# MeshFEM/MeshFEM

Measured on AMD Instinct MI355X. Metric: stiffness_assembly_elements_per_s, higher is better.
Workload: dtype f64

## Files before the change

### meshfem_amd/csrc/mfh_api.cpp

```cpp
#include "mfh_ctx.hh"
#include <dlfcn.h>

using namespace mfh;

namespace {
struct RoctxApi {
    int (*push)(const char *) = nullptr;
    int (*pop)() = nullptr;
    RoctxApi() {
        const char *en = getenv("MFH_ROCTX");
        if (!en || en[0] == '0') return;
        for (const char *lib : {"librocprofiler-sdk-roctx.so", "libroctx64.so", "/opt/rocm/lib/librocprofiler-sdk-roctx.so", "/opt/rocm/lib/libroctx64.so"}) {
            if (void *h = dlopen(lib, RTLD_NOW | RTLD_GLOBAL)) {
                push = reinterpret_cast<int (*)(const char *)>(dlsym(h, "roctxRangePushA"));
                pop = reinterpret_cast<int (*)()>(dlsym(h, "roctxRangePop"));
                if (push && pop) return;
                push = nullptr; pop = nullptr;
            }
        }
    }
};
RoctxApi &roctx_api() { static RoctxApi a; return a; }
}
mfh::RoctxRange::RoctxRange(const char *name) {
// ... 67 lines not shown
void upload_mesh(mfh_ctx *c, bool deviceTables) {
    double t0 = now_ms();
    c->autoStretch = -1.0;
    drop_p1_view(c);
    c->opDegree = 0;
    c->nodePairsValid = false;
    if (!c->hostOnly && !deviceTables) {
        require_device(c);
        MFH_HIP(hipSetDevice(c->device));
        c->dElemNodes.upload(c->mesh.elemNodes, c->stream);
        c->dVertPos.upload(c->mesh.nodePos, c->stream);
    }
    c->timing.upload_ms = now_ms() - t0;
    c->haveMesh = true;
    c->external = false;
    c->geoValid = false;
    c->hGeoValid = false;
    c->dofForNode.clear();
    c->nDoF = c->mesh.nNode;
    build_shape_tables(c->mesh.dim, c->mesh.deg, c->tables);
    if (!c->hostOnly) { c->dPairTable.upload(c->tables.pairTable, c->stream); c->dMassTable.upload(c->tables.massRef, c->stream); }
    invalidate_symbolic(c);
    dist_detach(c);
    reset_bcs(c);
    clear_fixed(c);
}

void set_isotropic(mfh_ctx *c, double E, double nu) {
    double lam = (nu * E) / ((1.0 + nu) * (1.0 - 2.0 * nu));
    if (c->haveMesh && c->mesh.dim == 2) lam = (nu * E) / (1.0 - nu * nu);
    c->matMode = 0;
    c->matKind = MAT_ISO;
    c->matParams = {lam, E / (2.0 + 2.0 * nu), E, nu};
    c->geoValid = false;
    c->hGeoValid = false;
    invalidate_matrix(c);
}

void drop_p1_view(mfh_ctx *c) {
    if (c->p1) { mfh_destroy(c->p1); c->p1 = nullptr; }
    c->p1GeoGen = -1;
}

mfh_ctx *p1_view(mfh_ctx *c) {
    if (!c || c->opDegree != 1 || !c->p1) return nullptr;
    mfh_ctx *v = c->p1;
    if (!c->hostOnly) {
        ensure_geometry(c);
        v->dGeo.borrow(c->dGeo.p, c->dGeo.n);
        v->geoStride = c->geoStride;
        v->geoValid = true;
        if (v->dVertPos.borrowed || !v->dVertPos.p) v->dVertPos.borrow(c->dVertPos.p, (size_t)v->mesh.nNode * v->mesh.dim);
        if (c->p1GeoGen != c->geoGen) { invalidate_matrix(v); c->p1GeoGen = c->geoGen; }
    }
    return v;
}

void ensure_pass_events(mfh_ctx *c) {
    if (c->passEv[0]) return;
    for (auto &e : c->passEv) MFH_HIP(hipEventCreate(&e));
    MFH_HIP(hipHostMalloc((void **)&c->negHost, 2 * sizeof(int), hipHostMallocDefault));
}

void ensure_geometry(mfh_ctx *c, bool deferCheck) {
    require(c->haveMesh, MFH_ERR_STATE, "no mesh set");
    if (c->geoValid) return;
    require(!c->hostOnly, MFH_ERR_HIP, "host-only context (device -1): no HIP device, and there is no CPU fallback");
    require_device(c);
    MFH_HIP(hipSetDevice(c->device));
    const HostMesh &m = c->mesh;
    if (c->matParams.empty() && !c->dMatBorrowed) set_isotropic(c, 1.0, 0.3);
    if (c->matMode == 0 && !c->dMatBorrowed) {
        double E = c->matParams[2], nu = c->matParams[3];
        double lam = (nu * E) / ((1.0 + nu) * (1.0 - 2.0 * nu));
        if (m.dim == 2) lam = (nu * E) / (1.0 - nu * nu);
        c->matParams[0] = lam;
    }
    c->geoStride = c->matKind == MAT_ISO ? GEO_ISO_STRIDE : (c->matKind == MAT_ORTHO ? GEO_ORTHO_STRIDE : GEO_GEN_STRIDE);
    if (!c->dMatBorrowed) c->dMatParams.upload(c->matParams, c->stream);
    const double *dMat = c->dMatBorrowed ? c->dMatBorrowed : c->dMatParams.p;
    c->dGeo.alloc((size_t)m.nElem * c->geoStride);
    c->dNeg.alloc(2);
    c->dNeg.zero(c->stream);
    ensure_pass_events(c);
    MFH_HIP(hipEventRecord(c->passEv[0], c->stream));
    k::launch_geometry(m.dim, m.deg, c->matKind, m.nElem, c->dElemNodes.p, m.npe, c->dVertPos.p, dMat, c->matMode,
                       c->dGeo.p, c->geoStride, c->dNeg.p, c->stream);
    MFH_HIP(hipEventRecord(c->passEv[1], c->stream));
    MFH_HIP(hipMemcpyAsync(c->negHost, c->dNeg.p, 2 * sizeof(int), hipMemcpyDeviceToHost, c->stream));
    c->geoPending = true;
    if (!deferCheck) finish_geometry(c);
}

void finish_geometry(mfh_ctx *c) {
    if (!c->geoPending) return;
    c->geoPending = false;
    MFH_HIP(hipStreamSynchronize(c->stream));
    float ms = 0;
    MFH_HIP(hipEventElapsedTime(&ms, c->passEv[0], c->passEv[1]));
    c->timing.geometry_ms = ms;
    const int neg[2] = {c->negHost[0], c->negHost[1]};
    if (neg[0] > 0)
        throw Error(MFH_ERR_INVALID, "Mesh has negatively oriented elements.\nCorrect with: mesh_convert --reorientNegativeElements. (" +
                                         std::to_string(neg[0]) + " elements)");
    if (neg[1] > 0)
        throw Error(MFH_ERR_INVALID, std::string(c->matMode == 1 ? "Isotropic" : "Orthotropic") + " parameters of " + std::to_string(neg[1]) +
                                         " elements give an indefinite elasticity tensor (" +
                                         (c->matMode == 1 ? "need E > 0 and -1 < nu < 1/2, nu < 1 in plane stress" : "compliance matrix not positive definite") + ").");
    c->geoValid = true;
    c->hGeoValid = false;
    ++c->geoGen;
}

const std::vector<double> &host_geo(mfh_ctx *c) {
    ensure_geometry(c);
    if (!c->hGeoValid) {
        c->hGeo.resize(c->dGeo.n);
        c->dGeo.download(c->hGeo.data(), c->dGeo.n, c->stream);
        c->hGeoValid = true;
    }
    return c->hGeo;
}

const int32_t *device_dof_map(mfh_ctx *c) {
    if (c->dofForNode.empty()) return nullptr;
    if (!c->dofUploaded) { c->dDofForNode.upload(c->dofForNode, c->stream); c->dofUploaded = true; }
    return c->dDofForNode.p;
}

void ensure_host_colidx(mfh_ctx *c) {
    if (!c->sym.colIdx.empty() || c->sym.nnzb == 0) return;
    c->sym.colIdx.resize((size_t)c->sym.nnzb);
    c->dColIdx.download(c->sym.colIdx.data(), c->sym.colIdx.size(), c->stream);
}
// ... 1009 lines not shown
    MFH_TRY(c)
    require(c && out, MFH_ERR_INVALID, "null argument");
    const std::vector<double> &g = host_geo(c);
    for (int64_t e = 0; e < c->mesh.nElem; ++e) out[e] = g[(size_t)e * c->geoStride + 12];
    MFH_CATCH(c)
}

mfh_status mfh_material_isotropic(mfh_ctx *c, double E, double nu) {
    MFH_TRY(c)
    require(c, MFH_ERR_INVALID, "null context");
    set_isotropic(c, E, nu);
    MFH_CATCH(c)
}

mfh_status mfh_material_const(mfh_ctx *c, const double *D) {
    MFH_TRY(c)
    require(c && D && c->haveMesh, MFH_ERR_STATE, "set the mesh before the material");
    const int d = c->dim(), fl = flat_len(d);
    c->matParams.clear();
    bool ortho = true;
    for (int r = 0; r < fl && ortho; ++r)
        for (int cc = r + 1; cc < fl; ++cc)
            if (cc >= d && D[r * fl + cc] != 0.0) { ortho = false; break; }
    if (ortho) {
        for (int r = 0; r < d; ++r)
            for (int cc = r; cc < d; ++cc) c->matParams.push_back(D[r * fl + cc]);
        for (int k2 = d; k2 < fl; ++k2) c->matParams.push_back(D[k2 * fl + k2]);
        c->matMode = 5; c->matKind = MAT_ORTHO;
    } else {
        for (int r = 0; r < fl; ++r)
            for (int cc = r; cc < fl; ++cc) c->matParams.push_back(D[r * fl + cc]);
        c->matMode = 2; c->matKind = MAT_GENERAL;
    }
    c->geoValid = false; c->hGeoValid = false;
    invalidate_matrix(c);
    MFH_CATCH(c)
}

mfh_status mfh_material_iso_field(mfh_ctx *c, const double *E, const double *nu) {
    MFH_TRY(c)
    require(c && E && nu && c->haveMesh, MFH_ERR_STATE, "set the mesh before the material");
    const int64_t n = c->mesh.nElem;
    c->matParams.assign((size_t)2 * n, 0.0);
    std::copy(E, E + n, c->matParams.begin());
    std::copy(nu, nu + n, c->matParams.begin() + n);
    c->matMode = 1; c->matKind = MAT_ISO;
    c->geoValid = false; c->hGeoValid = false;
    invalidate_matrix(c);
    MFH_CATCH(c)
}

mfh_status mfh_material_ortho_field(mfh_ctx *c, const double *params) {
    MFH_TRY(c)
    require(c && params && c->haveMesh, MFH_ERR_STATE, "set the mesh before the material");
    const int np = c->dim() == 3 ? 9 : 4;
    c->matParams.assign(params, params + (size_t)np * c->mesh.nElem);
    c->matMode = 3; c->matKind = MAT_ORTHO;
    c->geoValid = false; c->hGeoValid = false;
    invalidate_matrix(c);
    MFH_CATCH(c)
}

mfh_status mfh_material_tensor_field(mfh_ctx *c, const double *D) {
    MFH_TRY(c)
    require(c && D && c->haveMesh, MFH_ERR_STATE, "set the mesh before the material");
    const int fl = flat_len(c->dim());
    c->matParams.assign(D, D + (size_t)fl * fl * c->mesh.nElem);
    c->matMode = 4; c->matKind = MAT_GENERAL;
    c->geoValid = false; c->hGeoValid = false;
    invalidate_matrix(c);
    MFH_CATCH(c)
}

mfh_status mfh_material_get(mfh_ctx *c, int64_t elem, double *D) {
    MFH_TRY(c)
    require(c && D && c->haveMesh && elem >= 0 && elem < c->mesh.nElem, MFH_ERR_INVALID, "bad element");
    const std::vector<double> &g = host_geo(c);
    elem_D(c, &g[(size_t)elem * c->geoStride], D);
    MFH_CATCH(c)
}

mfh_status mfh_dof_map(mfh_ctx *c, const int32_t *dofForNode, int64_t nDoF) {
    MFH_TRY(c)
    require(!(c && c->opDegree == 1 && c->p1), MFH_ERR_STATE, "a forced-degree-1 view is in force (mfh_set_operator_degree): it is defined for the identity DoF map");
    require(c && c->haveMesh, MFH_ERR_STATE, "no mesh set");
    c->nOwnedDoFSet = -1;
    if (!dofForNode) {
        c->dofForNode.clear();
        c->nDoF = c->mesh.nNode;
        std::fill(c->mesh.bdryInternal.begin(), c->mesh.bdryInternal.end(), (uint8_t)0);
    } else {
        require(c->mesh.nOwned == c->mesh.nNode, MFH_ERR_UNSUPPORTED, "a DoF map on a partitioned mesh says which DoFs are this rank's rows: mfh_dof_map_partitioned");
        require(nDoF > 0 && nDoF <= c->mesh.nNode, MFH_ERR_INVALID, "bad nDoF");
        for (int64_t n = 0; n < c->mesh.nNode; ++n)
            require(dofForNode[n] >= 0 && dofForNode[n] < nDoF, MFH_ERR_INVALID, "DoF index out of range");
        c->dofForNode.assign(dofForNode, dofForNode + c->mesh.nNode);
        c->nDoF = nDoF;
    }
    invalidate_symbolic(c);
    clear_fixed(c);
    MFH_CATCH(c)
// ... 58 lines not shown

mfh_status mfh_symbolic_get(const mfh_ctx *c, int32_t *rowPtr, int32_t *colIdx, int32_t *chunkRow, int64_t *contribPtr,
                            uint32_t *contribCode, uint16_t *contribSlot, int32_t *scatterSlot) {
    if (c && c->opDegree == 1 && c->p1) return mfh_symbolic_get(c->p1, rowPtr, colIdx, chunkRow, contribPtr, contribCode, contribSlot, scatterSlot);
    if (!c || !c->symValid) return MFH_ERR_STATE;
    const Symbolic &S = c->sym;
    if (rowPtr) std::copy(S.rowPtr.begin(), S.rowPtr.end(), rowPtr);
    if (colIdx) std::copy(S.colIdx.begin(), S.colIdx.end(), colIdx);
    if (chunkRow) std::copy(S.chunkRow.begin(), S.chunkRow.end(), chunkRow);
    if (contribPtr) std::copy(S.contribPtr.begin(), S.contribPtr.end(), contribPtr);
    if (contribCode || contribSlot || scatterSlot) {
        if (S.contribCode.empty()) return MFH_ERR_STATE;
        if (contribCode) std::copy(S.contribCode.begin(), S.contribCode.end(), contribCode);
        if (contribSlot) std::copy(S.contribSlot.begin(), S.contribSlot.end(), contribSlot);
        if (scatterSlot) {
            if (S.scatterSlot.empty()) return MFH_ERR_STATE;
            std::copy(S.scatterSlot.begin(), S.scatterSlot.end(), scatterSlot);
        }
    }
    return MFH_OK;
}

mfh_status mfh_assemble(mfh_ctx *c, int32_t mode) {
    { mfh_status st; if (follow_view(c, st, [&](mfh_ctx *v) { return mfh_assemble(v, mode); })) return st; }
    MFH_TRY(c)
    require(c && c->haveMesh, MFH_ERR_STATE, "no mesh set");
    require(mode == MFH_ASSEMBLE_GATHER || mode == MFH_ASSEMBLE_ATOMIC, MFH_ERR_INVALID, "bad assembly mode");
    require(!(c->deterministic && mode == MFH_ASSEMBLE_ATOMIC), MFH_ERR_UNSUPPORTED, "option deterministic: the global-atomic assembly variant is not reproducible");
    if (c->alwaysReembed) { c->geoValid = false; c->hGeoValid = false; }
    ensure_symbolic(c, mode == MFH_ASSEMBLE_ATOMIC);
    RoctxRange range("Assemble System");
    ensure_geometry(c, true);
    ensure_pass_events(c);
    MFH_HIP(hipEventRecord(c->passEv[2], c->stream));
    run_assembly(c, mode);
    MFH_HIP(hipEventRecord(c->passEv[3], c->stream));
    if (c->geoPending) finish_geometry(c);
    else MFH_HIP(hipStreamSynchronize(c->stream));
    float ms = 0;
    MFH_HIP(hipEventElapsedTime(&ms, c->passEv[2], c->passEv[3]));
    c->timing.assemble_ms = ms;
    if (mode == MFH_ASSEMBLE_GATHER && c->placementTrials > 0 && c->placementGen != c->valsGen) placement_trials(c);
    c->assembled = true;
    c->dinvValid = false;
    MFH_CATCH(c)
}

mfh_status mfh_matrix_info(const mfh_ctx *c, int64_t *nBlockRows, int64_t *nBlockCols, int64_t *nnzBlocks) {
    if (c && c->opDegree == 1 && c->p1) return mfh_matrix_info(c->p1, nBlockRows, nBlockCols, nnzBlocks);
    if (!c || !c->symValid) return MFH_ERR_STATE;
    if (nBlockRows) *nBlockRows = c->sym.nRows;
    if (nBlockCols) *nBlockCols = c->sym.nCols;
    if (nnzBlocks) *nnzBlocks = c->sym.nnzb + (c->upperOnly ? c->sym.nMirror : 0);
    return MFH_OK;
}

mfh_status mfh_matrix_storage(const mfh_ctx *c, int32_t *upperOnly, int64_t *storedBlocks) {
    if (c && c->opDegree == 1 && c->p1) return mfh_matrix_storage(c->p1, upperOnly, storedBlocks);
    if (!c || !c->symValid) return MFH_ERR_STATE;
    if (upperOnly) *upperOnly = c->upperOnly ? 1 : 0;
    if (storedBlocks) *storedBlocks = c->sym.nnzb;
    return MFH_OK;
}

mfh_status mfh_matrix_set_upper_triplets(mfh_ctx *c, int64_t n, int64_t nnz, const uint64_t *ti, const uint64_t *tj, const double *tv) {
    MFH_TRY(c)
    require(c && n > 0 && nnz >= 0 && (nnz == 0 || (ti && tj && tv)), MFH_ERR_INVALID, "bad matrix arguments");
    require(n < (int64_t)1 << 31, MFH_ERR_UNSUPPORTED, "matrix too large for 32-bit indices");
    require(nnz < ((int64_t)1 << 30), MFH_ERR_UNSUPPORTED, "matrix has too many non-zeros for 32-bit slots (2 nnz must stay below 2^31)");
    require_device(c);
    MFH_HIP(hipSetDevice(c->device));
    struct Ent { int32_t r, c; double v; };
    std::vector<Ent> ent;
// ... 786 lines not shown
```

### meshfem_amd/csrc/mfh_ctx.hh

```
#pragma once
#include "mfh_internal.hh"
#include <cmath>
#include <map>
#include <mutex>

using namespace mfh;

struct mfh_ctx {
    int device = 0;
    bool hostOnly = false;
    bool hierarchyLevel = false;
    bool keepHostSymbolic = false;
    int xcdSwizzle = 0;
    RawVec<double> hLoad, hX, hXBatch, hLoadBatch;
    bool alwaysReembed = false;
    bool deterministic = false;
    DBuf<double> detPartials;
    DBuf<unsigned> detCounter;
    bool periodicIgnoreMismatch = false;
    int periodicIgnoreDims = 0;
    hipStream_t stream = nullptr;
    bool ownStream = true;
    bool arenaCounted = false;
    std::string err;

    HostMesh mesh;
    bool haveMesh = false;
    bool external = false;
    DBuf<int32_t> dElemNodes;
    DBuf<double> dVertPos;

    int matMode = 0;
    int matKind = MAT_ISO;
    int op = MFH_OP_ELASTICITY;
    int opDegree = 0;
    mfh_ctx *p1 = nullptr;
    int64_t geoGen = 0, p1GeoGen = -1;
    DBuf<int32_t> dNodePtr, dNodePair;
    bool nodePairsValid = false;
    std::vector<double> matParams;
    DBuf<double> dMatParams;
    const double *dMatBorrowed = nullptr;
    DBuf<double> dGeo;
    DBuf<int> dNeg;
    int geoStride = GEO_ISO_STRIDE;
    bool geoValid = false;
    hipEvent_t passEv[4] = {nullptr, nullptr, nullptr, nullptr};
    int *negHost = nullptr;
    bool geoPending = false;
    std::vector<double> hGeo;
    bool hGeoValid = false;

    std::vector<int32_t> dofForNode;
    DBuf<int32_t> dDofForNode;
    bool dofUploaded = false;
    int64_t nDoF = 0;

    Symbolic sym;
    bool symValid = false;
    bool symHasScatter = false;
    DBuf<int32_t> dRowPtr, dColIdx, dChunkRow, dSpmvChunkRow, dScatter;
    DBuf<int64_t> dContribPtr;
    int matrixStorage = -1;
    bool upperOnly = false;
    int nCU = 256;
    DBuf<uint32_t> dContribCode;
    DBuf<uint16_t> dContribSlot;
    ShapeTables tables;
    DBuf<double> dPairTable, dMassTable;
    MfLists mf;
    bool mfValid = false;
    int matrixFree = -1;
    bool use_mf() const {
        if (external || !haveMesh || hostOnly || kron()) return false;
        return matrixFree == 1 || (matrixFree < 0 && op == MFH_OP_ELASTICITY);
    }
    DBuf<int32_t> dMfChunkRow;
    DBuf<int64_t> dMfPairPtr;
    DBuf<uint32_t> dMfPairCode, dMfPairPos;
    DBuf<uint16_t> dMfPairRow;
    MfClusterLists mfc;
// ... 242 lines not shown
}

inline bool resolve_upper_storage(const mfh_ctx *c) {
    if (c->matrixStorage >= 0) return c->matrixStorage == 1;
    return c->haveMesh && !c->hostOnly && !c->external && c->op == MFH_OP_ELASTICITY && c->use_mf() && !c->tlProbe && c->tlRapAgg;
}

inline void require_full_storage(const mfh_ctx *c, const char *what) {
    if (c->upperOnly) throw Error(MFH_ERR_UNSUPPORTED, std::string(what) + " needs both triangles of K: set option matrix_storage to 0");
}

inline int32_t dof_of(const mfh_ctx *c, int64_t node) { return c->dofForNode.empty() ? (int32_t)node : c->dofForNode[node]; }
void invalidate_matrix(mfh_ctx *c);
void ensure_dirichlet_tables(mfh_ctx *c);
void dist_detach(mfh_ctx *c);
bool dist_active(const mfh_ctx *c);
int dist_rank(const mfh_ctx *c);
int dist_world(const mfh_ctx *c);
void dist_apply(mfh_ctx *c, double *x, double *y, bool masked);
void dist_halo(mfh_ctx *c, double *v, int W);
void dist_allreduce(mfh_ctx *c, double *dev, int64_t n);
void dist_level_forward(mfh_ctx *c, mfh_ctx::AggLevel &A, double *v, int W);
void dist_level_reverse_add(mfh_ctx *c, mfh_ctx::AggLevel &A, double *v, int W);
void dist_exchange_lists(mfh_ctx *c, const std::vector<std::vector<int32_t>> &toRank, std::vector<std::vector<int32_t>> &fromRank);
void dist_setup_child(mfh_ctx *c, mfh_ctx *child, const std::vector<int32_t> &keep);
void dist_agree(mfh_ctx *c);
void dist_profile_collect(mfh_ctx *c);
void refresh_storage_rule(mfh_ctx *c);
void reset_bcs(mfh_ctx *c);
void clear_fixed(mfh_ctx *c);
void add_fixed(mfh_ctx *c, int64_t n, const int64_t *vars, const double *vals);
void ensure_geometry(mfh_ctx *c, bool deferCheck = false);
void finish_geometry(mfh_ctx *c);
void ensure_node_pairs(mfh_ctx *c);
void ensure_mf_cluster(mfh_ctx *c);
void upload_mesh(mfh_ctx *c, bool deviceTables);
void ensure_fixed_uploaded(mfh_ctx *c);
bool prepare_matrix_free(mfh_ctx *c);
k::SpmvArgs spmv_args(mfh_ctx *c, bool masked);
k::SpmvMfArgs spmv_mf_args(mfh_ctx *c, bool masked);
k::SpmvMfArgs spmv_mf_cluster_args(mfh_ctx *c, bool masked);
k::TLArgs tl_args(mfh_ctx *c);
void apply_operator(mfh_ctx *c, bool masked, const double *x, double *y, double *dotOut);
void apply_operator_smoother(mfh_ctx *c, bool masked, const double *x, double *y);
void batch_apply(mfh_ctx *c, int NR, double *x, double *y, bool masked);
void tl_precond(mfh_ctx *c, const double *r, double *z, double *scal, int it);
bool dense_inverse_device(mfh_ctx *c, const double *Ac, int64_t mm, DBuf<double> &Ainv, int64_t &ldInv);
double device_dot(mfh_ctx *c, int64_t n, const double *a, const double *b);
void ensure_precond(mfh_ctx *c);
bool ensure_twolevel(mfh_ctx *c);
bool ensure_multigrid(mfh_ctx *c);
void ensure_coarse_levels(mfh_ctx *c, int nrhs);
void destroy_multigrid(mfh_ctx *c);
mfh_ctx *make_linear_context(mfh_ctx *c, int64_t nCN, const int32_t *coarseNode, bool borrowPositions);
mfh_ctx *p1_view(mfh_ctx *c);
void drop_p1_view(mfh_ctx *c);
struct MgFuse { bool presmoothed = false; double *rzScal = nullptr; const uint8_t *rzMask = nullptr; };
const float *smoother_dinv32(mfh_ctx *c);
double mg_fuse_scale(const mfh_ctx *c);
void mg_precond(mfh_ctx *c, const double *r, double *z, const double *scal, int it, const double *stop, const MgFuse *fuse = nullptr);
void mg_precond_batch(mfh_ctx *c, int NR, const double *r, double *z, int64_t vecStride, const double *scal, int64_t scalStride, int it, const double *stop,
                      const MgFuse *fuse = nullptr);
k::AsmArgs asm_args(mfh_ctx *c);
const int32_t *device_dof_map(mfh_ctx *c);
void box_corners(mfh_ctx *c, const double *mn, const double *mx, int relative, double *omn, double *omx);
void dirichlet_vars(mfh_ctx *c, std::vector<int64_t> &vars, std::vector<double> &vals);
// ... 15 lines not shown
```

### meshfem_amd/csrc/mfh_kernels.hip

```cpp
#include "mfh_device.hh"

namespace mfh { namespace k {

template <int DIM, int MAT> DEV constexpr int mat_nb() { return (MAT == MAT_LAPLACE || MAT == MAT_MASS) ? 1 : DIM * DIM; }

template <int DIM, int MAT>
DEV void block_from_H(const double *__restrict__ g, const double (&H)[DIM][DIM], double *K);

template <int DIM>
DEV void pair_H(const double *__restrict__ g, uint32_t offs , double S0, double S1, double S2,
                double S3, double (&H)[DIM][DIM]) {
#ifndef MFH_ASM_ABLATE
#define MFH_ASM_ABLATE 0
#endif
    const double vol = MFH_ASM_ABLATE >= 1 ? 1.0 : g[12];
    S0 *= vol; S1 *= vol; S2 *= vol; S3 *= vol;
    const char *gb = reinterpret_cast<const char *>(g);
    const double *gsi = reinterpret_cast<const double *>(gb + (offs & 0xffu)), *gti = reinterpret_cast<const double *>(gb + ((offs >> 8) & 0xffu)),
                 *gsj = reinterpret_cast<const double *>(gb + ((offs >> 16) & 0xffu)), *gtj = reinterpret_cast<const double *>(gb + (offs >> 24));
    double ua[DIM], ub[DIM], p[DIM], q[DIM];
#pragma unroll
    for (int a = 0; a < DIM; ++a) {
        ua[a] = MFH_ASM_ABLATE >= 1 ? S0 + a : gsi[a]; ub[a] = MFH_ASM_ABLATE >= 1 ? S1 - a : gti[a];
        const double va = MFH_ASM_ABLATE >= 2 ? S2 + a : gsj[a], vb = MFH_ASM_ABLATE >= 2 ? S3 - a : gtj[a];
// ... 183 lines not shown
            const double c00 = a11 * a22 - a12 * a12, c01 = a02 * a12 - a01 * a22, c02 = a01 * a12 - a02 * a11;
            const double c11 = a00 * a22 - a02 * a02, c12 = a01 * a02 - a00 * a12, c22 = a00 * a11 - a01 * a01;
            const double det = a00 * c00 + a01 * c01 + a02 * c02;
            if (!(a00 > 0 && c22 > 0 && det > 0 && q[6] > 0 && q[7] > 0 && q[8] > 0)) atomicAdd(negCount + 1, 1);
            g[13 + npack<3>(0, 0)] = c00 / det; g[13 + npack<3>(0, 1)] = c01 / det; g[13 + npack<3>(0, 2)] = c02 / det;
            g[13 + npack<3>(1, 1)] = c11 / det; g[13 + npack<3>(1, 2)] = c12 / det; g[13 + npack<3>(2, 2)] = c22 / det;
            g[ortho_shear_offset<3>() + 0] = q[6]; g[ortho_shear_offset<3>() + 1] = q[7]; g[ortho_shear_offset<3>() + 2] = q[8];
        } else {
            const double *q = mp + e * 4;
            const double a00 = 1.0 / q[0], a01 = -q[2] / q[1], a11 = 1.0 / q[1];
            const double det = a00 * a11 - a01 * a01;
            if (!(a00 > 0 && det > 0 && q[3] > 0)) atomicAdd(negCount + 1, 1);
            g[13 + npack<2>(0, 0)] = a11 / det; g[13 + npack<2>(0, 1)] = -a01 / det; g[13 + npack<2>(1, 1)] = a00 / det;
            g[ortho_shear_offset<2>()] = q[3];
        }
    } else {
        const double *q = mp + e * FL * FL;
        for (int r = 0; r < FL; ++r)
            for (int c = r; c < FL; ++c) g[13 + dpack<DIM>(r, c)] = q[r * FL + c];
    }
    }
    __syncthreads();
    const int64_t e0 = (int64_t)blockIdx.x * blockDim.x;
    const int nLive = (int)(nElem - e0 < (int64_t)blockDim.x ? nElem - e0 : (int64_t)blockDim.x);
    double *out = geo + e0 * stride;
    for (int q = threadIdx.x; q < nLive * stride; q += blockDim.x) {
        const int el = q / stride;
        out[q] = recs[(size_t)el * (stride + 1) + (q - el * stride)];
    }
}

template <int DIM, int DEG, int MAT> DEV constexpr bool asm_uses_table() { return DEG == 2 && MAT != MAT_MASS; }
constexpr int ASM_CODE_SHIFT = 7;

template <int DIM, int DEG, int MAT, bool UPPER = false, bool DET = false>
__global__ void __launch_bounds__(256, (MAT == MAT_GENERAL || MAT == MAT_ORTHO) ? 1 : 8) k_assemble_gather(AsmArgs a) {
    constexpr int NB = mat_nb<DIM, MAT>();
    constexpr int NPE = (DIM == 3) ? (DEG == 1 ? 4 : 10) : (DEG == 1 ? 3 : 6);
    constexpr bool TAB = asm_uses_table<DIM, DEG, MAT>();
    extern __shared__ __attribute__((aligned(16))) double acc[];
    const int CS = a.chunkSlots + 2;
    double *tabS = acc + (size_t)NB * CS;
    uint32_t *tabO = reinterpret_cast<uint32_t *>(tabS + NPE * NPE * 4);
    uint32_t *turn = tabO + NPE * NPE;
    const PairConst pc{a.pairConst[0], a.pairConst[1], a.pairConst[2], a.pairConst[3], a.pairConst[4], a.pairConst[5]};
    const int64_t item = a.xcd == 1 ? xcd_item(blockIdx.x, gridDim.x) : (a.xcd > 1 ? xcd_group_item(blockIdx.x, gridDim.x, a.xcd) : (int64_t)blockIdx.x);
    const int64_t chunk = a.chunkOrder ? (int64_t)a.chunkOrder[item] : item;
    const int r0 = a.chunkRow[chunk], r1 = a.chunkRow[chunk + 1];
    const int s0 = a.rowPtr[r0];
    const int ns = a.rowPtr[r1] - s0;
    const uint32_t eBase = a.chunkElemBase ? (uint32_t)a.chunkElemBase[chunk] : 0u;
    const int par = s0 & 1;
    for (int t = threadIdx.x; t < ns + par; t += 256)
#pragma unroll
        for (int c = 0; c < NB; ++c) acc[c * CS + t] = 0.0;
    if (DET && threadIdx.x == 0) *turn = 0u;
    if (TAB) {
        for (int t = threadIdx.x; t < NPE * NPE; t += 256) {
            const int i = t / NPE, j = t - i * NPE;
#pragma unroll
            for (int k = 0; k < 4; ++k) tabS[t * 4 + k] = a.pairTable[t * 4 + k];
            tabO[t] = (uint32_t)(sup_s<DIM, DEG>(i) * DIM * 8) | ((uint32_t)(sup_t<DIM, DEG>(i) * DIM * 8) << 8) |
                      ((uint32_t)(sup_s<DIM, DEG>(j) * DIM * 8) << 16) | ((uint32_t)(sup_t<DIM, DEG>(j) * DIM * 8) << 24);
        }
    }
    __syncthreads();
    const int64_t kb = a.contribPtr[chunk], ke = a.contribPtr[chunk + 1];
    constexpr int U = 2;
    constexpr bool det = DET;
    unsigned turnNo = threadIdx.x >> 6;
    for (int64_t k0 = kb + threadIdx.x; det ? (k0 - threadIdx.x < ke) : (k0 < ke); k0 += 256 * U) {
        uint32_t code[U];
        int ls[U];
        bool ok[U];
#pragma unroll
        for (int u = 0; u < U; ++u) {
            const int64_t kk = k0 + (int64_t)u * 256;
            ok[u] = kk < ke;
            code[u] = ok[u] ? a.contribCode[kk] : a.contribCode[kb];
            ls[u] = (ok[u] ? (int)a.contribSlot[kk] : 0) + par;
        }
#pragma unroll
        for (int u = 0; u < U; ++u) {
            double K[NB];
            if (ok[u]) {
            uint32_t e;
            int ij;
            if (a.chunkElemBase) { e = eBase + (code[u] >> ASM_CODE_SHIFT); ij = (int)(code[u] & ((1u << ASM_CODE_SHIFT) - 1)); }
            else { e = code[u] / (NPE * NPE); ij = (int)(code[u] - e * (NPE * NPE)); }
            const double *g = a.geo + (int64_t)e * a.geoStride;
            if (TAB) {
                typedef double dv2 __attribute__((ext_vector_type(2)));
                const dv2 s01 = *reinterpret_cast<const dv2 *>(&tabS[ij * 4]), s23 = *reinterpret_cast<const dv2 *>(&tabS[ij * 4 + 2]);
                const uint32_t offs = tabO[ij];
                double H[DIM][DIM];
                pair_H<DIM>(g, offs, s01.x, s01.y, s23.x, s23.y, H);
                block_from_H<DIM, MAT>(g, H, K);
            } else {
                const int i = ij / NPE, j = ij - i * NPE;
                elem_block<DIM, DEG, MAT>(g, MAT == MAT_MASS ? a.massTable : a.pairTable, pc, i, j, K);
            }
            }
            if (det) {
                if ((threadIdx.x & 63) == 0)
                    while (__hip_atomic_load(turn, __ATOMIC_ACQUIRE, __HIP_MEMORY_SCOPE_WORKGROUP) != turnNo) __builtin_amdgcn_s_sleep(1);
                if (ok[u]) {
#pragma unroll
                    for (int c = 0; c < NB; ++c) unsafeAtomicAdd(&acc[c * CS + ls[u]], K[c]);
                }
                __builtin_amdgcn_fence(__ATOMIC_RELEASE, "workgroup");
                if ((threadIdx.x & 63) == 0) __hip_atomic_store(turn, turnNo + 1u, __ATOMIC_RELEASE, __HIP_MEMORY_SCOPE_WORKGROUP);
                turnNo += 4u;
            } else if (ok[u]) {
#pragma unroll
                for (int c = 0; c < NB; ++c) unsafeAtomicAdd(&acc[c * CS + ls[u]], K[c]);
            }
            __builtin_amdgcn_sched_barrier(0);
        }
    }
    __syncthreads();
    const int nl = ns + par;
    const int64_t sbase = (int64_t)s0 - par;
    const int pfirst = par;
    const int plast = nl >> 1;
    for (int p = pfirst + threadIdx.x; p < plast; p += 256) {
        const int t = 2 * p;
        const int64_t s = sbase + t;
#pragma unroll
        for (int c = 0; c < NB; ++c) {
// ... 1931 lines not shown
        const int key_ = (a.dim == 3 ? 0 : 6) + (a.deg == 2 ? 3 : 0) + (a.mat == MAT_GENERAL ? 1 : (a.mat == MAT_ORTHO ? 2 : 0)); \
        switch (key_) {                                                                  \
        case 0: { CALL(3, 1, MAT_ISO); } break;                                           \
        case 1: { CALL(3, 1, MAT_GENERAL); } break;                                       \
        case 2: { CALL(3, 1, MAT_ORTHO); } break;                                         \
        case 3: { CALL(3, 2, MAT_ISO); } break;                                           \
        case 4: { CALL(3, 2, MAT_GENERAL); } break;                                       \
        case 5: { CALL(3, 2, MAT_ORTHO); } break;                                         \
        case 6: { CALL(2, 1, MAT_ISO); } break;                                           \
        case 7: { CALL(2, 1, MAT_GENERAL); } break;                                       \
        case 8: { CALL(2, 1, MAT_ORTHO); } break;                                         \
        case 9: { CALL(2, 2, MAT_ISO); } break;                                           \
        case 10: { CALL(2, 2, MAT_GENERAL); } break;                                      \
        default: { CALL(2, 2, MAT_ORTHO); } break;                                        \
        }                                                                                \
    } while (0)

#define MFH_DISPATCH_ASM(a, CALL)                                                        \
    do {                                                                                 \
        if (!mat_is_scalar(a.mat)) { MFH_DISPATCH(a, CALL); break; }                     \
        const int key_ = (a.dim == 3 ? 0 : 4) + (a.deg == 2 ? 2 : 0) + (a.mat == MAT_MASS ? 1 : 0); \
        switch (key_) {                                                                  \
        case 0: { CALL(3, 1, MAT_LAPLACE); } break;                                       \
        case 1: { CALL(3, 1, MAT_MASS); } break;                                          \
        case 2: { CALL(3, 2, MAT_LAPLACE); } break;                                       \
        case 3: { CALL(3, 2, MAT_MASS); } break;                                          \
        case 4: { CALL(2, 1, MAT_LAPLACE); } break;                                       \
        case 5: { CALL(2, 1, MAT_MASS); } break;                                          \
        case 6: { CALL(2, 2, MAT_LAPLACE); } break;                                       \
        default: { CALL(2, 2, MAT_MASS); } break;                                         \
        }                                                                                \
    } while (0)

void launch_assemble_gather(const AsmArgs &a, hipStream_t s) {
    if (a.nChunk == 0) return;
    size_t lds = (size_t)(mat_is_scalar(a.mat) ? 1 : a.dim * a.dim) * (a.chunkSlots + 2) * sizeof(double);
    if (a.deg == 2 && a.mat != MAT_MASS) lds += (size_t)a.npe * a.npe * (4 * sizeof(double) + sizeof(uint32_t));
    if (a.det) lds = (size_t)(mat_is_scalar(a.mat) ? 1 : a.dim * a.dim) * (a.chunkSlots + 2) * sizeof(double) + (size_t)a.npe * a.npe * (4 * sizeof(double) + sizeof(uint32_t)) + 16;
#define CALLV(D, G, M, UP, DT)                                                                                 \
    do {                                                                                                         \
        if (lds > 64 * 1024)                                                                                     \
            MFH_HIP(hipFuncSetAttribute((const void *)k_assemble_gather<D, G, M, UP, DT>, hipFuncAttributeMaxDynamicSharedMemorySize, (int)lds)); \
        hipLaunchKernelGGL((k_assemble_gather<D, G, M, UP, DT>), dim3((unsigned)a.nChunk), dim3(256), lds, s, a); \
    } while (0)
#define CALL(D, G, M)                                                     \
    if (a.det) { if (a.upperOnly) CALLV(D, G, M, true, true); else CALLV(D, G, M, false, true); } \
    else { if (a.upperOnly) CALLV(D, G, M, true, false); else CALLV(D, G, M, false, false); }
    MFH_DISPATCH_ASM(a, CALL);
#undef CALL
#undef CALLV
    CHECK_LAUNCH();
}

void launch_chunk_keys(const AsmArgs &a, uint32_t *keys, hipStream_t s) {
    if (a.nChunk == 0) return;
    hipLaunchKernelGGL(k_chunk_keys, dim3((unsigned)((a.nChunk + 255) / 256)), dim3(256), 0, s, a.nChunk, a.contribPtr, a.contribCode,
                       a.chunkElemBase, (uint32_t)(a.npe * a.npe), keys);
    CHECK_LAUNCH();
}

bool launch_pack_codes(int64_t nChunk, const int64_t *contribPtr, uint32_t *contribCode, int npe, int32_t *chunkElemBase, int *flag, hipStream_t s) {
    if (nChunk == 0) return true;
    MFH_HIP(hipMemsetAsync(flag, 0, sizeof(int), s));
    hipLaunchKernelGGL(k_pack_codes, dim3((unsigned)nChunk), dim3(64), 0, s, nChunk, contribPtr, contribCode, (uint32_t)(npe * npe), chunkElemBase, flag, 0);
    CHECK_LAUNCH();
    int h = 0;
    MFH_HIP(hipMemcpyAsync(&h, flag, sizeof(int), hipMemcpyDeviceToHost, s));
    MFH_HIP(hipStreamSynchronize(s));
    if (h) return false;
    hipLaunchKernelGGL(k_pack_codes, dim3((unsigned)nChunk), dim3(64), 0, s, nChunk, contribPtr, contribCode, (uint32_t)(npe * npe), chunkElemBase, flag, 1);
    CHECK_LAUNCH();
    return true;
}

void launch_assemble_atomic(const AsmArgs &a, hipStream_t s) {
// ... 442 lines not shown
```

### meshfem_amd/csrc/mfh_multigrid.cpp

```cpp
#include "mfh_ctx.hh"

namespace mfhi {

namespace {

struct LevelOps {
    int64_t n = 0;
    std::function<void(const double *, double *)> apply;
    std::function<void(const double *rin, const double *t, double *rout, double *d, double *x, double a, double b, bool first, bool assign)> step;
    std::function<void(double *)> mask;
    std::function<void(double *, int64_t)> reduce;
    double lmax = 0, ratio = 0.3;
    int steps = 1;
};

LevelOps nodal_ops(mfh_ctx *c, const double *scal, int it, const double *stop, int NR = 1) {
    LevelOps L;
    const int d = c->bs();
    const int64_t nRows = c->sym.nRows;
    const bool masked = !c->fixedVars.empty();
    hipStream_t s = c->stream;
    L.n = nRows * d * NR;
    if (NR > 1) {
        L.apply = [=](const double *x, double *y) { batch_apply(c, NR, const_cast<double *>(x), y, masked); };
// ... 711 lines not shown
    lap("vertices, coarse DoFs, parents");
    resPtr.assign((size_t)nCD + 1, 0);
    for (int64_t f = 0; f < nDoF; ++f)
        if (parA[(size_t)f] >= 0 && coarseDofOfFine[(size_t)f] < 0) { ++resPtr[(size_t)parA[(size_t)f] + 1]; ++resPtr[(size_t)parB[(size_t)f] + 1]; }
    for (int64_t q = 0; q < nCD; ++q) resPtr[(size_t)q + 1] += resPtr[(size_t)q];
    resIdx.assign((size_t)resPtr[(size_t)nCD], 0);
    std::vector<int32_t> cur(resPtr.begin(), resPtr.end() - 1);
    for (int64_t f = 0; f < nDoF; ++f)
        if (parA[(size_t)f] >= 0 && coarseDofOfFine[(size_t)f] < 0) {
            resIdx[(size_t)cur[(size_t)parA[(size_t)f]]++] = (int32_t)f;
            resIdx[(size_t)cur[(size_t)parB[(size_t)f]]++] = (int32_t)f;
        }
    lap("restriction lists");
    }
    auto coarse_node = [&](int64_t n) -> int32_t { return ownNumbering ? (n < m.nVert ? (int32_t)n : -1) : coarseNode[(size_t)n]; };
    auto coarse_dof = [&](int64_t f) -> int32_t { return ownNumbering ? (f < m.nVert ? (int32_t)f : -1) : coarseDofOfFine[(size_t)f]; };
    mfh_ctx *c1 = make_linear_context(c, nCN, ownNumbering ? nullptr : coarseNode.data(), false);
    G.coarse = c1;
    HostMesh &m1 = c1->mesh;
    int64_t nOwnedCoarseDoF = -1;
    if (distributed && c->dofForNode.empty()) {
        int64_t nOwnedCoarse = 0;
        for (int64_t n = 0; n < m.nOwned; ++n) nOwnedCoarse += coarse_node(n) >= 0;
        m1.nOwned = nOwnedCoarse;
    } else if (distributed) {
        nOwnedCoarseDoF = 0;
        for (int64_t f = 0; f < c->nOwnedDoF(); ++f) nOwnedCoarseDoF += coarse_dof(f) >= 0;
    }
    lap("linear mesh + upload");
    c1->matMode = c->matMode; c1->matKind = c->matKind;
    if (c->matParams.size() > 64) {
        ensure_geometry(c);
        c1->dMatBorrowed = c->dMatParams.p;
    } else c1->matParams = c->matParams;
    c1->geoValid = false;
    if (nCD != nCN || nOwnedCoarseDoF >= 0) {
        c1->dofForNode.assign((size_t)nCN, 0);
        for (int64_t n = 0; n < m.nNode; ++n)
            if (coarse_node(n) >= 0) c1->dofForNode[(size_t)coarse_node(n)] = coarse_dof(dof_of(c, n));
        c1->nDoF = nCD;
        c1->nOwnedDoFSet = nOwnedCoarseDoF;
        c1->dofUploaded = false;
    }
    {
        std::vector<int64_t> fv;
        for (int64_t v : c->fixedVars) {
            const int64_t f = v / d;
            if (coarse_dof(f) >= 0) fv.push_back((int64_t)coarse_dof(f) * d + v % d);
        }
        clear_fixed(c1);
        if (!fv.empty()) add_fixed(c1, (int64_t)fv.size(), fv.data(), nullptr);
    }
    c1->matrixFree = 0;
    c1->matrixStorage = 0;
    c1->aggNodes = c->mgAggNodes;
    c1->precond = distributed ? MFH_PRECOND_BLOCK_JACOBI : MFH_PRECOND_TWO_LEVEL;
    if (distributed) dist_setup_child(c, c1, c->dofForNode.empty() ? coarseNode : coarseDofOfFine);
    lap("linear level: material, DoF map, fixed variables");
    ensure_precond(c1);
    make_fp32_copy(c, c1, distributed);
    lap("linear level: symbolic + assembly");
    bool haveCoarse = build_aggregate_hierarchy(c, c1, lap);
    if (!haveCoarse && !distributed && !singular) {
        haveCoarse = ensure_twolevel(c1);
        lap("linear level: rigid-body coarse (dense)");
    }
    G.nFine = c->sym.nRows; G.nCoarse = c1->sym.nRows;
// ... 175 lines not shown
```

Before: 1.642 billion.

## Halve assembly pair table in LDS and skip redundant material uploads

Stores only the upper-triangular node-pair shape table in LDS, with per-node offsets, and mirrors entries for the lower triangle. This cuts LDS per workgroup, which may allow more resident workgroups. Material parameters are now uploaded only when a generation counter changes, and the negative-element counter buffer is kept across calls and diffed, which drops a per-call memset and memcpy. Assembly timing now spans from the geometry end event, and an optional residency report is added behind an environment variable.

After: 1.537 billion. 0.936x the previous value.

```diff
diff --git a/meshfem_amd/csrc/mfh_api.cpp b/meshfem_amd/csrc/mfh_api.cpp
--- a/meshfem_amd/csrc/mfh_api.cpp
+++ b/meshfem_amd/csrc/mfh_api.cpp
@@ -123,6 +123,7 @@
     c->matMode = 0;
     c->matKind = MAT_ISO;
     c->matParams = {lam, E / (2.0 + 2.0 * nu), E, nu};
+    ++c->matGen;
     c->geoValid = false;
     c->hGeoValid = false;
     invalidate_matrix(c);
@@ -165,32 +166,48 @@
         double E = c->matParams[2], nu = c->matParams[3];
         double lam = (nu * E) / ((1.0 + nu) * (1.0 - 2.0 * nu));
         if (m.dim == 2) lam = (nu * E) / (1.0 - nu * nu);
-        c->matParams[0] = lam;
+        if (c->matParams[0] != lam) { c->matParams[0] = lam; ++c->matGen; }
     }
     c->geoStride = c->matKind == MAT_ISO ? GEO_ISO_STRIDE : (c->matKind == MAT_ORTHO ? GEO_ORTHO_STRIDE : GEO_GEN_STRIDE);
-    if (!c->dMatBorrowed) c->dMatParams.upload(c->matParams, c->stream);
+    if (!c->dMatBorrowed && (c->matUploadedGen != c->matGen || c->dMatParams.n != c->matParams.size())) {
+        c->dMatParams.upload(c->matParams, c->stream);
+        c->matUploadedGen = c->matGen;
+    }
     const double *dMat = c->dMatBorrowed ? c->dMatBorrowed : c->dMatParams.p;
     c->dGeo.alloc((size_t)m.nElem * c->geoStride);
-    c->dNeg.alloc(2);
-    c->dNeg.zero(c->stream);
     ensure_pass_events(c);
+    if (c->geoPending) read_geometry_counters(c);
+    if (!c->dNeg.p) {
+        c->dNeg.alloc(2);
+        c->dNeg.zero(c->stream);
+        c->negSeen[0] = c->negSeen[1] = 0u;
+    }
     MFH_HIP(hipEventRecord(c->passEv[0], c->stream));
     k::launch_geometry(m.dim, m.deg, c->matKind, m.nElem, c->dElemNodes.p, m.npe, c->dVertPos.p, dMat, c->matMode,
                        c->dGeo.p, c->geoStride, c->dNeg.p, c->stream);
     MFH_HIP(hipEventRecord(c->passEv[1], c->stream));
-    MFH_HIP(hipMemcpyAsync(c->negHost, c->dNeg.p, 2 * sizeof(int), hipMemcpyDeviceToHost, c->stream));
     c->geoPending = true;
     if (!deferCheck) finish_geometry(c);
+}
+
+void read_geometry_counters(mfh_ctx *c, unsigned *counted) {
+    MFH_HIP(hipMemcpyAsync(c->negHost, c->dNeg.p, 2 * sizeof(int), hipMemcpyDeviceToHost, c->stream));
+    MFH_HIP(hipStreamSynchronize(c->stream));
+    for (int k2 = 0; k2 < 2; ++k2) {
+        const unsigned now = (unsigned)c->negHost[k2];
+        if (counted) counted[k2] = now - c->negSeen[k2];
+        c->negSeen[k2] = now;
+    }
 }
 
 void finish_geometry(mfh_ctx *c) {
     if (!c->geoPending) return;
     c->geoPending = false;
-    MFH_HIP(hipStreamSynchronize(c->stream));
+    unsigned neg[2] = {0u, 0u};
+    read_geometry_counters(c, neg);
     float ms = 0;
     MFH_HIP(hipEventElapsedTime(&ms, c->passEv[0], c->passEv[1]));
     c->timing.geometry_ms = ms;
-    const int neg[2] = {c->negHost[0], c->negHost[1]};
     if (neg[0] > 0)
         throw Error(MFH_ERR_INVALID, "Mesh has negatively oriented elements.\nCorrect with: mesh_convert --reorientNegativeElements. (" +
                                          std::to_string(neg[0]) + " elements)");
@@ -1266,6 +1283,7 @@
             for (int cc = r; cc < fl; ++cc) c->matParams.push_back(D[r * fl + cc]);
         c->matMode = 2; c->matKind = MAT_GENERAL;
     }
+    ++c->matGen;
     c->geoValid = false; c->hGeoValid = false;
     invalidate_matrix(c);
     MFH_CATCH(c)
@@ -1279,6 +1297,7 @@
     std::copy(E, E + n, c->matParams.begin());
     std::copy(nu, nu + n, c->matParams.begin() + n);
     c->matMode = 1; c->matKind = MAT_ISO;
+    ++c->matGen;
     c->geoValid = false; c->hGeoValid = false;
     invalidate_matrix(c);
     MFH_CATCH(c)
@@ -1290,6 +1309,7 @@
     const int np = c->dim() == 3 ? 9 : 4;
     c->matParams.assign(params, params + (size_t)np * c->mesh.nElem);
     c->matMode = 3; c->matKind = MAT_ORTHO;
+    ++c->matGen;
     c->geoValid = false; c->hGeoValid = false;
     invalidate_matrix(c);
     MFH_CATCH(c)
@@ -1301,6 +1321,7 @@
     const int fl = flat_len(c->dim());
     c->matParams.assign(D, D + (size_t)fl * fl * c->mesh.nElem);
     c->matMode = 4; c->matKind = MAT_GENERAL;
+    ++c->matGen;
     c->geoValid = false; c->hGeoValid = false;
     invalidate_matrix(c);
     MFH_CATCH(c)
@@ -1425,13 +1446,13 @@
     RoctxRange range("Assemble System");
     ensure_geometry(c, true);
     ensure_pass_events(c);
+    if (!c->geoPending) MFH_HIP(hipEventRecord(c->passEv[1], c->stream));
+    run_assembly(c, mode);
     MFH_HIP(hipEventRecord(c->passEv[2], c->stream));
-    run_assembly(c, mode);
-    MFH_HIP(hipEventRecord(c->passEv[3], c->stream));
     if (c->geoPending) finish_geometry(c);
     else MFH_HIP(hipStreamSynchronize(c->stream));
     float ms = 0;
-    MFH_HIP(hipEventElapsedTime(&ms, c->passEv[2], c->passEv[3]));
+    MFH_HIP(hipEventElapsedTime(&ms, c->passEv[1], c->passEv[2]));
     c->timing.assemble_ms = ms;
     if (mode == MFH_ASSEMBLE_GATHER && c->placementTrials > 0 && c->placementGen != c->valsGen) placement_trials(c);
     c->assembled = true;
diff --git a/meshfem_amd/csrc/mfh_ctx.hh b/meshfem_amd/csrc/mfh_ctx.hh
--- a/meshfem_amd/csrc/mfh_ctx.hh
+++ b/meshfem_amd/csrc/mfh_ctx.hh
@@ -40,13 +40,15 @@
     bool nodePairsValid = false;
     std::vector<double> matParams;
     DBuf<double> dMatParams;
+    int64_t matGen = 0, matUploadedGen = -1;
     const double *dMatBorrowed = nullptr;
     DBuf<double> dGeo;
     DBuf<int> dNeg;
     int geoStride = GEO_ISO_STRIDE;
     bool geoValid = false;
-    hipEvent_t passEv[4] = {nullptr, nullptr, nullptr, nullptr};
+    hipEvent_t passEv[3] = {nullptr, nullptr, nullptr};
     int *negHost = nullptr;
+    unsigned negSeen[2] = {0u, 0u};
     bool geoPending = false;
     std::vector<double> hGeo;
     bool hGeoValid = false;
@@ -355,6 +357,7 @@
 void add_fixed(mfh_ctx *c, int64_t n, const int64_t *vars, const double *vals);
 void ensure_geometry(mfh_ctx *c, bool deferCheck = false);
 void finish_geometry(mfh_ctx *c);
+void read_geometry_counters(mfh_ctx *c, unsigned *counted = nullptr);
 void ensure_node_pairs(mfh_ctx *c);
 void ensure_mf_cluster(mfh_ctx *c);
 void upload_mesh(mfh_ctx *c, bool deviceTables);
diff --git a/meshfem_amd/csrc/mfh_kernels.hip b/meshfem_amd/csrc/mfh_kernels.hip
--- a/meshfem_amd/csrc/mfh_kernels.hip
+++ b/meshfem_amd/csrc/mfh_kernels.hip
@@ -239,17 +239,19 @@
 
 template <int DIM, int DEG, int MAT> DEV constexpr bool asm_uses_table() { return DEG == 2 && MAT != MAT_MASS; }
 constexpr int ASM_CODE_SHIFT = 7;
+static inline size_t asm_table_bytes(int npe) { return (size_t)(npe * (npe + 1) / 2) * 4 * sizeof(double) + (size_t)npe * sizeof(uint32_t); }
 
 template <int DIM, int DEG, int MAT, bool UPPER = false, bool DET = false>
 __global__ void __launch_bounds__(256, (MAT == MAT_GENERAL || MAT == MAT_ORTHO) ? 1 : 8) k_assemble_gather(AsmArgs a) {
     constexpr int NB = mat_nb<DIM, MAT>();
     constexpr int NPE = (DIM == 3) ? (DEG == 1 ? 4 : 10) : (DEG == 1 ? 3 : 6);
     constexpr bool TAB = asm_uses_table<DIM, DEG, MAT>();
+    constexpr int NPAIR = NPE * (NPE + 1) / 2;
     extern __shared__ __attribute__((aligned(16))) double acc[];
     const int CS = a.chunkSlots + 2;
     double *tabS = acc + (size_t)NB * CS;
-    uint32_t *tabO = reinterpret_cast<uint32_t *>(tabS + NPE * NPE * 4);
-    uint32_t *turn = tabO + NPE * NPE;
+    uint32_t *tabO = reinterpret_cast<uint32_t *>(tabS + NPAIR * 4);
+    uint32_t *turn = tabO + NPE;
     const PairConst pc{a.pairConst[0], a.pairConst[1], a.pairConst[2], a.pairConst[3], a.pairConst[4], a.pairConst[5]};
     const int64_t item = a.xcd == 1 ? xcd_item(blockIdx.x, gridDim.x) : (a.xcd > 1 ? xcd_group_item(blockIdx.x, gridDim.x, a.xcd) : (int64_t)blockIdx.x);
     const int64_t chunk = a.chunkOrder ? (int64_t)a.chunkOrder[item] : item;
@@ -265,10 +267,12 @@
     if (TAB) {
         for (int t = threadIdx.x; t < NPE * NPE; t += 256) {
             const int i = t / NPE, j = t - i * NPE;
-#pragma unroll
-            for (int k = 0; k < 4; ++k) tabS[t * 4 + k] = a.pairTable[t * 4 + k];
-            tabO[t] = (uint32_t)(sup_s<DIM, DEG>(i) * DIM * 8) | ((uint32_t)(sup_t<DIM, DEG>(i) * DIM * 8) << 8) |
-                      ((uint32_t)(sup_s<DIM, DEG>(j) * DIM * 8) << 16) | ((uint32_t)(sup_t<DIM, DEG>(j) * DIM * 8) << 24);
+            if (i <= j) {
+                const int r = ((i * (2 * NPE + 1 - i)) >> 1) + (j - i);
+#pragma unroll
+                for (int k = 0; k < 4; ++k) tabS[r * 4 + k] = a.pairTable[t * 4 + k];
+            }
+            if (t < NPE) tabO[t] = (uint32_t)(sup_s<DIM, DEG>(t) * DIM * 8) | ((uint32_t)(sup_t<DIM, DEG>(t) * DIM * 8) << 8);
         }
     }
     __syncthreads();
@@ -298,10 +302,14 @@
             const double *g = a.geo + (int64_t)e * a.geoStride;
             if (TAB) {
                 typedef double dv2 __attribute__((ext_vector_type(2)));
-                const dv2 s01 = *reinterpret_cast<const dv2 *>(&tabS[ij * 4]), s23 = *reinterpret_cast<const dv2 *>(&tabS[ij * 4 + 2]);
-                const uint32_t offs = tabO[ij];
+                const int i = ij / NPE, j = ij - i * NPE;
+                const bool mirrored = i > j;
+                const int lo = mirrored ? j : i, hi = mirrored ? i : j;
+                const int r = ((lo * (2 * NPE + 1 - lo)) >> 1) + (hi - lo);
+                const dv2 s01 = *reinterpret_cast<const dv2 *>(&tabS[r * 4]), s23 = *reinterpret_cast<const dv2 *>(&tabS[r * 4 + 2]);
+                const uint32_t offs = tabO[i] | (tabO[j] << 16);
                 double H[DIM][DIM];
-                pair_H<DIM>(g, offs, s01.x, s01.y, s23.x, s23.y, H);
+                pair_H<DIM>(g, offs, s01.x, mirrored ? s23.x : s01.y, mirrored ? s01.y : s23.x, s23.y, H);
                 block_from_H<DIM, MAT>(g, H, K);
             } else {
                 const int i = ij / NPE, j = ij - i * NPE;
@@ -2299,15 +2307,33 @@
         }                                                                                \
     } while (0)
 
+static void report_residency(const void *fn, const char *name, size_t lds) {
+    int nb = 0, nbMore = 0;
+    MFH_HIP(hipOccupancyMaxActiveBlocksPerMultiprocessor(&nb, fn, 256, lds));
+    size_t upTo = lds;
+    for (size_t more = lds + 64; more <= lds + 8192 && more <= 64 * 1024; more += 64) {
+        MFH_HIP(hipOccupancyMaxActiveBlocksPerMultiprocessor(&nbMore, fn, 256, more));
+        if (nbMore != nb) break;
+        upTo = more;
+    }
+    fprintf(stderr, "[assembly] %s: %zu B of LDS per workgroup, %d resident workgroups per CU (the same up to %zu B)\n", name, lds, nb, upTo);
+}
+
 void launch_assemble_gather(const AsmArgs &a, hipStream_t s) {
     if (a.nChunk == 0) return;
     size_t lds = (size_t)(mat_is_scalar(a.mat) ? 1 : a.dim * a.dim) * (a.chunkSlots + 2) * sizeof(double);
-    if (a.deg == 2 && a.mat != MAT_MASS) lds += (size_t)a.npe * a.npe * (4 * sizeof(double) + sizeof(uint32_t));
-    if (a.det) lds = (size_t)(mat_is_scalar(a.mat) ? 1 : a.dim * a.dim) * (a.chunkSlots + 2) * sizeof(double) + (size_t)a.npe * a.npe * (4 * sizeof(double) + sizeof(uint32_t)) + 16;
+    if (a.deg == 2 && a.mat != MAT_MASS) lds += asm_table_bytes(a.npe);
+    if (a.det) lds = (size_t)(mat_is_scalar(a.mat) ? 1 : a.dim * a.dim) * (a.chunkSlots + 2) * sizeof(double) + asm_table_bytes(a.npe) + 16;
+    static const bool report = getenv("MFH_ASM_TIMING") != nullptr;
 #define CALLV(D, G, M, UP, DT)                                                                                 \
     do {                                                                                                         \
         if (lds > 64 * 1024)                                                                                     \
             MFH_HIP(hipFuncSetAttribute((const void *)k_assemble_gather<D, G, M, UP, DT>, hipFuncAttributeMaxDynamicSharedMemorySize, (int)lds)); \
+        static bool reported = false;                                                                            \
+        if (report && !reported) {                                                                               \
+            reported = true;                                                                                     \
+            report_residency((const void *)k_assemble_gather<D, G, M, UP, DT>, "k_assemble_gather<" #D "," #G "," #M "," #UP "," #DT ">", lds); \
+        }                                                                                                        \
         hipLaunchKernelGGL((k_assemble_gather<D, G, M, UP, DT>), dim3((unsigned)a.nChunk), dim3(256), lds, s, a); \
     } while (0)
 #define CALL(D, G, M)                                                     \
diff --git a/meshfem_amd/csrc/mfh_multigrid.cpp b/meshfem_amd/csrc/mfh_multigrid.cpp
--- a/meshfem_amd/csrc/mfh_multigrid.cpp
+++ b/meshfem_amd/csrc/mfh_multigrid.cpp
@@ -767,7 +767,7 @@
     if (c->matParams.size() > 64) {
         ensure_geometry(c);
         c1->dMatBorrowed = c->dMatParams.p;
-    } else c1->matParams = c->matParams;
+    } else { c1->matParams = c->matParams; ++c1->matGen; }
     c1->geoValid = false;
     if (nCD != nCN || nOwnedCoarseDoF >= 0) {
         c1->dofForNode.assign((size_t)nCN, 0);
```
